# apple/ml-stable-diffusion

Measured on NVIDIA H100. Metric: diffusion_iter_per_s, higher is better.
Workload: dtype f16

## Files before the change

### ml-stable-diffusion_b200/csrc/common.cuh

```cuda
#pragma once

#include <cuda.h>
#include <cuda_fp16.h>
#include <cuda_runtime.h>
#include <stdint.h>
#include <stdio.h>
#include <string.h>

namespace b200sd {

void set_error(const char* fmt, ...);

#define B200SD_CHECK_CUDA(expr)                                                            \
    do {                                                                                   \
        cudaError_t _e = (expr);                                                           \
        if (_e != cudaSuccess) {                                                           \
            ::b200sd::set_error("%s failed: %s (%s:%d)", #expr, cudaGetErrorString(_e),    \
                                __FILE__, __LINE__);                                       \
            return 1;                                                                      \
        }                                                                                  \
    } while (0)

#define B200SD_REQUIRE(cond, ...)                                                          \
    do {                                                                                   \
// ... 255 lines not shown
        : "memory");
}

__device__ __forceinline__ void wgmma_m64n64_rs_tb(float* d, const uint32_t (&a)[4], uint64_t db, uint32_t acc) {
    asm volatile(
        "{\n\t.reg .pred p;\n\tsetp.ne.b32 p, %37, 0;\n\t"
        "wgmma.mma_async.sync.aligned.m64n64k16.f32.f16.f16 "
        "{%0, %1, %2, %3, %4, %5, %6, %7, %8, %9, %10, %11, %12, %13, %14, %15, "
        "%16, %17, %18, %19, %20, %21, %22, %23, %24, %25, %26, %27, %28, %29, %30, %31}, "
        "{%32, %33, %34, %35}, %36, p, 1, 1, 1;\n\t}\n"
        : B200SD_F8(0), B200SD_F8(8), B200SD_F8(16), B200SD_F8(24)
        : "r"(a[0]), "r"(a[1]), "r"(a[2]), "r"(a[3]), "l"(db), "r"(acc)
        : "memory");
}
template <int N>
__device__ __forceinline__ void wgmma_rs_tb(float* d, const uint32_t (&a)[4], uint64_t db, uint32_t acc);
template <>
__device__ __forceinline__ void wgmma_rs_tb<64>(float* d, const uint32_t (&a)[4], uint64_t db, uint32_t acc) {
    wgmma_m64n64_rs_tb(d, a, db, acc);
}
template <>
__device__ __forceinline__ void wgmma_rs_tb<128>(float* d, const uint32_t (&a)[4], uint64_t db, uint32_t acc) {
    asm volatile(
        "{\n\t.reg .pred p;\n\tsetp.ne.b32 p, %69, 0;\n\t"
        "wgmma.mma_async.sync.aligned.m64n128k16.f32.f16.f16 "
        "{%0, %1, %2, %3, %4, %5, %6, %7, %8, %9, %10, %11, %12, %13, %14, %15, "
        "%16, %17, %18, %19, %20, %21, %22, %23, %24, %25, %26, %27, %28, %29, %30, %31, "
        "%32, %33, %34, %35, %36, %37, %38, %39, %40, %41, %42, %43, %44, %45, %46, %47, "
        "%48, %49, %50, %51, %52, %53, %54, %55, %56, %57, %58, %59, %60, %61, %62, %63}, "
        "{%64, %65, %66, %67}, %68, p, 1, 1, 1;\n\t}\n"
        : B200SD_F8(0), B200SD_F8(8), B200SD_F8(16), B200SD_F8(24), B200SD_F8(32), B200SD_F8(40), B200SD_F8(48), B200SD_F8(56)
        : "r"(a[0]), "r"(a[1]), "r"(a[2]), "r"(a[3]), "l"(db), "r"(acc)
        : "memory");
}
template <>
__device__ __forceinline__ void wgmma_rs_tb<192>(float* d, const uint32_t (&a)[4], uint64_t db, uint32_t acc) {
    asm volatile(
        "{\n\t.reg .pred p;\n\tsetp.ne.b32 p, %101, 0;\n\t"
        "wgmma.mma_async.sync.aligned.m64n192k16.f32.f16.f16 "
        "{%0, %1, %2, %3, %4, %5, %6, %7, %8, %9, %10, %11, %12, %13, %14, %15, "
        "%16, %17, %18, %19, %20, %21, %22, %23, %24, %25, %26, %27, %28, %29, %30, %31, "
        "%32, %33, %34, %35, %36, %37, %38, %39, %40, %41, %42, %43, %44, %45, %46, %47, "
        "%48, %49, %50, %51, %52, %53, %54, %55, %56, %57, %58, %59, %60, %61, %62, %63, "
        "%64, %65, %66, %67, %68, %69, %70, %71, %72, %73, %74, %75, %76, %77, %78, %79, "
        "%80, %81, %82, %83, %84, %85, %86, %87, %88, %89, %90, %91, %92, %93, %94, %95}, "
        "{%96, %97, %98, %99}, %100, p, 1, 1, 1;\n\t}\n"
        : B200SD_F8(0), B200SD_F8(8), B200SD_F8(16), B200SD_F8(24), B200SD_F8(32), B200SD_F8(40), B200SD_F8(48), B200SD_F8(56),
          B200SD_F8(64), B200SD_F8(72), B200SD_F8(80), B200SD_F8(88)
        : "r"(a[0]), "r"(a[1]), "r"(a[2]), "r"(a[3]), "l"(db), "r"(acc)
        : "memory");
}
#undef B200SD_F8

template <int R>
__device__ __forceinline__ void wgmma_rows64(float (&d)[R], int bn, uint64_t da, uint64_t db, uint32_t acc) {
#pragma unroll
    for (int c = 0; c + 64 <= 2 * R; c += 64)
        if (c + 64 <= bn) wgmma_ss<64>(d + c / 2, da, db + (c * 128 >> 4), acc);
    const int c32 = bn & ~63;
#pragma unroll
    for (int c = 0; c + 32 <= 2 * R; c += 64)
        if (c == c32 && (bn & 32)) wgmma_ss<32>(d + c / 2, da, db + (c * 128 >> 4), acc);
    const int c16 = bn & ~31;
#pragma unroll
    for (int c = 0; c + 16 <= 2 * R; c += 32)
        if (c == c16 && (bn & 16)) wgmma_ss<16>(d + c / 2, da, db + (c * 128 >> 4), acc);
}

__device__ __forceinline__ uint64_t make_smem_desc_sw128(uint32_t smem_addr, uint32_t sbo_bytes, uint32_t lbo_bytes) {
    uint64_t d = 0;
    d |= static_cast<uint64_t>((smem_addr >> 4) & 0x3FFF);
    d |= static_cast<uint64_t>((lbo_bytes >> 4) & 0x3FFF) << 16;
    d |= static_cast<uint64_t>((sbo_bytes >> 4) & 0x3FFF) << 32;
    d |= static_cast<uint64_t>(1) << 62;
    return d;
}

__device__ __forceinline__ float ex2_approx(float x) {
    float y;
    asm("ex2.approx.ftz.f32 %0, %1;" : "=f"(y) : "f"(x));
    return y;
}

__device__ __forceinline__ float silu_f(float x) { return __fdividef(x, 1.0f + __expf(-x)); }
__device__ __forceinline__ float erf_as(float x) {
    const float ax = fabsf(x);
    float t;
    asm("rcp.approx.ftz.f32 %0, %1;" : "=f"(t) : "f"(fmaf(0.3275911f, ax, 1.0f)));
    float poly = fmaf(1.061405429f, t, -1.453152027f);
    poly = fmaf(poly, t, 1.421413741f);
    poly = fmaf(poly, t, -0.284496736f);
    poly = fmaf(poly, t, 0.254829592f);
    poly *= t;
    const float e = ex2_approx(-ax * ax * 1.4426950408889634f);
    const float r = fmaf(-poly, e, 1.0f);
    return copysignf(r, x);
}
__device__ __forceinline__ float gelu_erf_f(float x) { return 0.5f * x * (1.0f + erf_as(x * 0.70710678118654752f)); }

__device__ __forceinline__ uint32_t pack_half2(float a, float b) {
    __half2 h = __floats2half2_rn(a, b);
    return *reinterpret_cast<uint32_t*>(&h);
}
#endif

}
```

### ml-stable-diffusion_b200/csrc/gemm_conv.cu

```cuda
#include "common.cuh"
#include "../../include/b200sd.h"

#include <algorithm>
#include <cmath>
#include <stdlib.h>

namespace b200sd {

static constexpr int kBM = 128;
static constexpr int kBK = 64;
static constexpr int kAStage = kBM * kBK * 2;
static constexpr int kGemmThreads = 384;
static constexpr int kProducerRegs = 40;
static constexpr int kConsumerRegs = 232;
static constexpr int kHaloThreads = 288;
static constexpr int kEpiThreads = 256;
static constexpr int kProducerWarp = 8;
static constexpr int kMaxStages = 8;
static constexpr int kHaloMaxStages = 24;
static constexpr int kSmemBudget = 220 * 1024;
static constexpr int kEpiFixed = 2 * 256 * 4 + 256 * 4 + 64;

static int smem_budget() {
    const char* e = getenv("B200SD_SMEM_KB");
    if (e && e[0]) {
        const int kb = atoi(e);
        if (kb >= 48 && kb <= 220) return kb * 1024;
    }
    return kSmemBudget;
}

struct __align__(64) GemmParams {
    CUtensorMap tmA0, tmA1, tmB;
    CUtensorMap tmA2, tmA3;
    int kc2, kc3;
    int mode, M, N, n_store;
    int C0, Kpt, kc0, kc, taps;
    int kb_total, kb_per_split, splits;
    int m_tiles, n_tiles, block_n, stages;
    int n_img, Hout, Wout, stride, bw_log2, bh_log2, tiles_w, tiles_h;
    int bias_rows, bias_stride, geglu, out_f32;
    int act;
    int cluster;
    int pad_lo;
    int wgt_tiled;
    int bias_mode;
    int res_smem;
    void* out;
    const float* bias;
    const __half* residual;
    float* partial;
    int H, W, Wp, tiles_per_img, patch_rows, patch_bytes, upsample;
    int inv_wp;
    int win, tw, th, tiles_x;
    int desc_bo;
    int tma_patch, patch_tx;
    const __half* a0;
    const __half* a1;
    int C1;
    const float* gn_chan0;
    const float* gn_chan1;
    const float* gn_gamma;
    const float* gn_beta;
    int gn_groups, gn_silu, gn_hw;
    float gn_eps;
    float* cs_partial;
    float* cs_chan;
    unsigned int* cs_tickets;
// ... 784 lines not shown
                                for (int j = 0; j < 16; ++j) a16[j] = __uint_as_float(v[j]);
                                process16(a16, c);
                            }
                        }
                    }
                    if (!kPartial && p.rs_out != nullptr && valid)
                        *reinterpret_cast<float2*>(p.rs_out + (static_cast<size_t>(t.n_tile * 2 + half) * p.M + out_row) * 2) = rowacc;
                }
            }
            fence_proxy_async_smem();
            epi_bar_sync();
            if (threadIdx.x == 0) mbar_arrive(acc_free);
        }
        if (kPartial && p.cluster) {
            cluster_sync_all();
            cluster_splitk_reduce(p, smem, threadIdx.x);
            cluster_sync_all();
        }
    }
}


static constexpr int kGemmWidths[] = {256, 192, 160, 128, 96, 64, 32, 16};
static constexpr int kNumGemmWidths = sizeof(kGemmWidths) / sizeof(kGemmWidths[0]);
static int gemm_width_index(int bn) {
    for (int i = 0; i < kNumGemmWidths; ++i)
        if (kGemmWidths[i] == bn) return i;
    return -1;
}
using KernelFn = void (*)(GemmParams);
template <bool kGeneric, bool kGeglu, bool kOutF32, bool kPartial, bool kStaged>
static KernelFn gemm_kernel(int width_index) {
#define B200SD_GEMM_FN(bn) wgmma_gemm_kernel<kGeneric, kGeglu, kOutF32, kPartial, kStaged, bn>
    static const KernelFn fns[kNumGemmWidths] = {B200SD_GEMM_FN(256), B200SD_GEMM_FN(192), B200SD_GEMM_FN(160),
                                                 B200SD_GEMM_FN(128), B200SD_GEMM_FN(96),  B200SD_GEMM_FN(64),
                                                 B200SD_GEMM_FN(32),  B200SD_GEMM_FN(16)};
#undef B200SD_GEMM_FN
    return fns[width_index];
}

__device__ __forceinline__ float silu_fast(float y) {
    float th;
    asm("tanh.approx.f32 %0, %1;" : "=f"(th) : "f"(0.5f * y));
    const float hy = 0.5f * y;
    return fmaf(hy, th, hy);
}

__device__ __forceinline__ void dbg_mark(const GemmParams& p, int slot) {
    if (p.dbg != nullptr && blockIdx.x == 0) p.dbg[slot] = clock64();
}

__device__ __forceinline__ void ldr_bar_sync() { asm volatile("bar.sync 1, 256;" ::: "memory"); }

template <int kKind, int kR>
__global__ void __launch_bounds__(kHaloThreads, 1) halo_conv_kernel(const __grid_constant__ GemmParams p) {
    constexpr bool kFp32Direct = kKind == 1;
    constexpr bool kTmaPatch = kKind == 2;
    extern __shared__ __align__(1024) uint8_t smem_raw[];
    uint8_t* smem = smem_raw;
    if (threadIdx.x == 0 && (smem_u32(smem) & 1023u) != 0) __trap();
    const int b_stage = p.block_n * (kBK * 2);
    uint8_t* patch = smem;
    uint8_t* smem_b = smem + 2 * p.patch_bytes;
    uint64_t* full_b = reinterpret_cast<uint64_t*>(smem_b + p.stages * b_stage);
    uint64_t* empty_b = full_b + kHaloMaxStages;
    uint64_t* full_a = empty_b + kHaloMaxStages;
    uint64_t* empty_a = full_a + 2;
    uint64_t* acc_free = empty_a + 2;
    float* bias_s = reinterpret_cast<float*>(acc_free + 4);
    unsigned int* flag_s = reinterpret_cast<unsigned int*>(bias_s + 256);
    float2* stat_s = reinterpret_cast<float2*>(flag_s + 16);
    float2* scsh = stat_s + 64;
    const int Cin = p.C0 + p.C1;
    __half* stage_tile = reinterpret_cast<__half*>(scsh + ((Cin + 7) & ~7));
    float* acc_s = reinterpret_cast<float*>(smem);
    const int lda = p.block_n + 4;

    const int warp = threadIdx.x >> 5;
    const int lane = threadIdx.x & 31;
    if (warp == kProducerWarp && lane == 0) {
        prefetch_tmap(&p.tmB);
        if (kTmaPatch) {
            prefetch_tmap(&p.tmA0);
            prefetch_tmap(&p.tmA1);
        }
        for (int s = 0; s < p.stages; ++s) {
            mbar_init(&full_b[s], 1);
            mbar_init(&empty_b[s], 2);
        }
        for (int s = 0; s < 2; ++s) {
            mbar_init(&full_a[s], 1);
            mbar_init(&empty_a[s], 2);
        }
        mbar_init(acc_free, 1);
        fence_barrier_init();
    }
    __syncthreads();
    pdl_trigger();

    const int total_work = p.m_tiles * p.n_tiles;
    const int work0 = blockIdx.x, work_step = gridDim.x;
    const int kc = p.kc;

    if (warp == kProducerWarp) {
        if (lane == 0) {
            int it = 0, iter = 0;
            int ci = 0, pai = 0, pwork = work0, pj = 0;
            auto issue_patch = [&](bool blocking) -> bool {
                const int pa = pai & 1;
                const uint32_t ph = ((pai >> 1) & 1) ^ 1;
                if (blocking) mbar_wait(&empty_a[pa], ph);
                else if (!mbar_try_wait(&empty_a[pa], ph)) return false;
                const TileCoord pt = decode_work(p, pwork);
                const bool src1 = pj >= p.kc0;
                mbar_expect_tx(&full_a[pa], static_cast<uint32_t>(p.patch_tx));
                tma_load_4d(patch + pa * p.patch_bytes + 1024, src1 ? &p.tmA1 : &p.tmA0, &full_a[pa],
                            (src1 ? pj - p.kc0 : pj) * kBK, pt.xa, pt.ya, pt.n0, kEvictNormal);
                ++pai;
                if (++pj == kc) pj = 0, pwork += work_step;
                return true;
            };
            if (kTmaPatch) pdl_wait();
            for (int work = work0; work < total_work; work += work_step, ++iter) {
                const TileCoord t = decode_work(p, work);
                if (iter > 0) mbar_wait(acc_free, (iter - 1) & 1);
                for (int j = 0; j < kc; ++j, ++ci) {
                    if (kTmaPatch && pai == ci) issue_patch(true);
                    for (int tap = 0; tap < p.taps; ++tap, ++it) {
                        if (kTmaPatch && pai == ci + 1 && pwork == work) issue_patch(false);
                        const int st = it % p.stages;
                        const uint32_t ph = (it / p.stages) & 1;
                        mbar_wait(&empty_b[st], ph ^ 1);
                        mbar_expect_tx(&full_b[st], b_stage);
                        tma_load_2d(smem_b + st * b_stage, &p.tmB, &full_b[st], 0,
                                    (t.n_tile * p.kb_total + j * p.taps + tap) * p.block_n, kEvictFirst);
                    }
                }
            }
        }
    } else if (warp < kProducerWarp) {
        const int ltid = threadIdx.x;
        const int ew = warp;
        const int wg = warp >> 2;
        const int r0 = 64 * wg + 16 * (warp & 3) + (lane >> 2);
        const int row = (warp & 3) * 32 + lane;
        const bool leader = (threadIdx.x & 127) == 0;
        const bool gn = p.gn_gamma != nullptr;
        const bool ups = p.upsample != 0;
        const int Hs = ups ? (p.H >> 1) : p.H, Ws = ups ? (p.W >> 1) : p.W;
        float acc[kR];
        if (ltid == 0) dbg_mark(p, 0);
        pdl_wait();
        if (ltid == 0) dbg_mark(p, 1);
        int cur_img = -1, ait = 0, it = 0;
        for (int work = work0; work < total_work; work += work_step) {
            const TileCoord t = decode_work(p, work);
            const int img = t.n0;
            const int ya = t.ya, xa = t.xa;
            const int ncol0 = t.n_tile * p.block_n;
            if (p.bias != nullptr) {
                const float* bsrc = p.bias + (p.bias_rows > 0 ? static_cast<size_t>(img) * p.bias_stride : 0);
                for (int c = ltid; c < p.block_n; c += kEpiThreads) bias_s[c] = (ncol0 + c < p.N) ? bsrc[ncol0 + c] : 0.f;
            }
            if (ltid < 16) {
                const int which = ltid >> 3;
                *reinterpret_cast<uint4*>(patch + which * p.patch_bytes + 7 * 128 + (ltid & 7) * 16) = make_uint4(0, 0, 0, 0);
            }
            constexpr int NBMAX = kTmaPatch ? 1 : 12;
            const int nvec = p.patch_rows * p.Wp * 8;
            const int nb = (nvec + kEpiThreads - 1) / kEpiThreads;
            const int jj = ltid & 7;
            int soff[NBMAX], doff[NBMAX];
            uint4 regs[NBMAX];
            auto chunk_src = [&](int j, int& csrc) -> const __half* {
                const bool src1 = j >= p.kc0;
                const int cbase = (src1 ? j - p.kc0 : j) * kBK + jj * 8;
                csrc = src1 ? p.C1 : p.C0;
                if (cbase >= csrc) return nullptr;
                return (src1 ? p.a1 : p.a0) + static_cast<size_t>(img) * Hs * Ws * csrc + cbase;
            };
            float4 cf[4];
            bool chan_ok = false;
            int csrc_nxt = 0;
            const __half* nsrc = nullptr;
            auto transform_begin = [&](int tj) {
                const bool src1 = tj >= p.kc0;
                int csrc_cur;
                chan_ok = chunk_src(tj, csrc_cur) != nullptr;
                nsrc = (tj + 1 < kc) ? chunk_src(tj + 1, csrc_nxt) : nullptr;
                if (gn) {
                    const float2* tab = scsh + (src1 ? p.C0 : 0) + (src1 ? tj - p.kc0 : tj) * kBK + jj * 8;
#pragma unroll
                    for (int q = 0; q < 4; ++q) cf[q] = chan_ok ? *reinterpret_cast<const float4*>(tab + 2 * q) : make_float4(0.f, 0.f, 0.f, 0.f);
                }
            };
            auto transform_slice = [&](int pa, int slice, int nslices) {
                uint8_t* pbase = patch + pa * p.patch_bytes + 1024;
#pragma unroll
                for (int i = 0; i < NBMAX; ++i) {
                    if (doff[i] < 0 || i % nslices != slice) continue;
                    uint4 val = regs[i];
                    const bool live = soff[i] >= 0;
                    regs[i] = make_uint4(0, 0, 0, 0);
                    if (nsrc != nullptr && live)
                        regs[i] = __ldg(reinterpret_cast<const uint4*>(nsrc + static_cast<size_t>(soff[i]) * csrc_nxt));
                    if (gn && live && chan_ok) {
                        __half2* h2 = reinterpret_cast<__half2*>(&val);
#pragma unroll
                        for (int q = 0; q < 4; ++q) {
                            const float2 f = __half22float2(h2[q]);
                            float a = fmaf(f.x, cf[q].x, cf[q].y), b = fmaf(f.y, cf[q].z, cf[q].w);
                            if (p.gn_silu) a = silu_fast(a), b = silu_fast(b);
                            h2[q] = __floats2half2_rn(a, b);
                        }
                    }
                    *reinterpret_cast<uint4*>(pbase + doff[i]) = val;
                }
            };
            if (!kTmaPatch) {
#pragma unroll
                for (int i = 0; i < NBMAX; ++i) {
                    const int v = ltid + kEpiThreads * i;
                    const int pi = v >> 3;
                    const int prow = (pi * p.inv_wp) >> 20;
                    const int yy = ya + prow, xx = xa + (pi - prow * p.Wp);
                    const bool in_patch = i < nb && v < nvec;
                    const bool ok = in_patch && yy >= 0 && yy < p.H && xx >= 0 && xx < p.W;
                    const int ys = ups ? (yy >> 1) : yy, xs = ups ? (xx >> 1) : xx;
                    soff[i] = ok ? (ys * Ws + xs) : -1;
                    doff[i] = in_patch ? pi * 128 + ((jj ^ (pi & 7)) << 4) : -1;
                }
                {
                    int csrc;
                    const __half* src = chunk_src(0, csrc);
#pragma unroll
                    for (int i = 0; i < NBMAX; ++i) {
                        regs[i] = make_uint4(0, 0, 0, 0);
                        if (src != nullptr && soff[i] >= 0)
                            regs[i] = __ldg(reinterpret_cast<const uint4*>(src + static_cast<size_t>(soff[i]) * csrc));
                    }
                }
                if (ltid == 0) dbg_mark(p, 2);
                if (gn && img != cur_img) {
                    const int cpg = Cin / p.gn_groups;
                    const float inv_cnt = 1.0f / (static_cast<float>(cpg) * static_cast<float>(p.gn_hw));
                    ldr_bar_sync();
                    for (int g = ltid >> 3; g < p.gn_groups; g += kEpiThreads >> 3) {
                        float s = 0.f, q = 0.f;
                        for (int c = g * cpg + (ltid & 7); c < (g + 1) * cpg; c += 8) {
                            const float2 v = (c < p.C0)
                                ? __ldg(reinterpret_cast<const float2*>(p.gn_chan0 + (static_cast<size_t>(img) * p.C0 + c) * 2))
                                : __ldg(reinterpret_cast<const float2*>(p.gn_chan1 + (static_cast<size_t>(img) * p.C1 + c - p.C0) * 2));
                            s += v.x, q += v.y;
                        }
#pragma unroll
                        for (int o = 4; o > 0; o >>= 1) {
                            s += __shfl_xor_sync(0xffffffffu, s, o);
                            q += __shfl_xor_sync(0xffffffffu, q, o);
                        }
                        if ((ltid & 7) == 0) {
                            const float mean = s * inv_cnt;
                            stat_s[g] = make_float2(mean, rsqrtf(fmaxf(q * inv_cnt - mean * mean, 0.f) + p.gn_eps));
                        }
                    }
                    ldr_bar_sync();
                    for (int c = ltid; c < Cin; c += kEpiThreads) {
                        const float2 st = stat_s[c / cpg];
                        const float sc = p.gn_gamma[c] * st.y;
                        scsh[c] = make_float2(sc, fmaf(-st.x, sc, p.gn_beta[c]));
                    }
                    ldr_bar_sync();
                    cur_img = img;
                }
                if (ltid == 0) dbg_mark(p, 8);
                transform_begin(0);
                transform_slice(ait & 1, 0, 1);
            }
            fence_proxy_async_smem();
            epi_bar_sync();
            if (ltid == 0) {
                if (!kTmaPatch) dbg_mark(p, 9);
                dbg_mark(p, 3);
            }
            for (int j = 0; j < kc; ++j, ++ait) {
                const int pa = ait & 1;
                if (kTmaPatch) mbar_wait(&full_a[pa], (ait >> 1) & 1);
                const bool more = !kTmaPatch && j + 1 < kc;
                if (ltid == 0 && j < 24) dbg_mark(p, 64 + 2 * j);
                if (more) {
                    if (ltid == 0 && j < 23) dbg_mark(p, 10 + 2 * j);
                    transform_begin(j + 1);
                }
                const uint32_t pbase = smem_u32(patch + pa * p.patch_bytes) + 1024;
                int prev = -1;
                for (int tap = 0; tap < p.taps; ++tap, ++it) {
                    const int st = it % p.stages;
                    mbar_wait(&full_b[st], (it / p.stages) & 1);
                    const int dy = p.taps == 9 ? tap / 3 - 1 : 0, dx = p.taps == 9 ? tap - (tap / 3) * 3 - 1 : 0;
                    const int srow = t.c0 + dy * p.Wp + dx + 64 * wg;
                    const uint32_t a_addr = pbase + srow * 128;
                    const uint64_t adesc = make_smem_desc_sw128(a_addr, 1024, 0) |
                                           (static_cast<uint64_t>(p.desc_bo ? ((a_addr >> 7) & 7) : 0) << 49);
                    const uint64_t bdesc = make_smem_desc_sw128(smem_u32(smem_b + st * b_stage), 1024, 0);
                    wgmma_fence();
#pragma unroll
                    for (int k = 0; k < kBK / 16; ++k)
                        wgmma_rows64(acc, p.block_n, adesc + 2 * k, bdesc + 2 * k, (j > 0 || tap > 0 || k > 0) ? 1u : 0u);
                    wgmma_commit();
                    if (more) transform_slice(pa ^ 1, tap, p.taps);
                    wgmma_wait<1>();
                    if (prev >= 0 && leader) mbar_arrive(&empty_b[prev]);
                    prev = st;
                }
                wgmma_wait<0>();
                wgmma_fence_regs<kR>(acc);
                if (ltid == 0 && j < 24) dbg_mark(p, 65 + 2 * j);
                if (leader) {
                    mbar_arrive(&empty_b[prev]);
                    if (kTmaPatch) mbar_arrive(&empty_a[pa]);
                }
                if (more) {
                    fence_proxy_async_smem();
                    epi_bar_sync();
                    if (ltid == 0 && j < 23) dbg_mark(p, 11 + 2 * j);
                }
            }
            int out_row;
            const bool valid = tile_row(p, t, row, out_row);
            uint4 res_pre[4];
            if (kKind == 0) staged_load_residual(p, t, staged_map(p, t, lane), ew, 0, res_pre);
            epi_bar_sync();
            if (ltid == 0) dbg_mark(p, 4);
            if (kKind == 0) {
                __half* tile_s = p.stage_dedicated ? stage_tile : reinterpret_cast<__half*>(smem);
                float* scratch = reinterpret_cast<float*>(tile_s + kBM * (p.block_n + 8));
                const float* bias = p.bias != nullptr ? bias_s : nullptr;
                stage_accumulators(p, t, acc, tile_s, bias, bias, bias_s, r0, lane);
                staged_epilogue(p, t, tile_s, scratch, flag_s, ew, lane, res_pre);
            } else {
                park_accumulators(acc, p.block_n, acc_s, lda, r0, lane);
                epi_bar_sync();
                const float* arow = acc_s + row * lda;
                if (kFp32Direct) {
                    if (ew < 4) {
                        uint32_t v[16];
                        acc_ld16(arow, v);
                        if (valid) {
                            for (int c = 0; c < 16 && ncol0 + c < p.N; ++c) {
                                const float x = __uint_as_float(v[c]) + (p.bias != nullptr ? bias_s[c] : 0.f);
                                if (p.out_f32) reinterpret_cast<float*>(p.out)[static_cast<size_t>(out_row) * p.N + ncol0 + c] = x;
                                else reinterpret_cast<__half*>(p.out)[static_cast<size_t>(out_row) * p.N + ncol0 + c] = __float2half_rn(x);
                            }
                        }
                    }
                } else {
                    const int half = ew >> 2;
                    float2 rowacc = make_float2(0.f, 0.f);
                    for (int c = 32 * half; c < p.block_n && valid; c += 64) {
                        uint32_t v[32];
                        acc_ld32(arow + c, v);
#pragma unroll
                        for (int hh = 0; hh < 2; ++hh) {
                            const int cc = c + 16 * hh;
                            if (ncol0 + cc < p.N) {
                                float a16[16];
#pragma unroll
                                for (int q = 0; q < 16; ++q) a16[q] = __uint_as_float(v[16 * hh + q]);
                                const float* bptr = p.bias != nullptr ? bias_s + cc : nullptr;
                                const __half* rptr = p.residual != nullptr
                                    ? p.residual + static_cast<size_t>(out_row) * p.n_store + ncol0 + cc : nullptr;
                                epilogue_store16<true, false, false, false>(p, a16, out_row, ncol0 + cc, 0, bptr, rptr, rowacc);
                            }
                        }
                    }
                }
            }
            fence_proxy_async_smem();
            epi_bar_sync();
            if (ltid == 0) {
                dbg_mark(p, 5);
                mbar_arrive(acc_free);
            }
        }
    }
}

__global__ void splitk_reduce_kernel(const float* __restrict__ partial, int splits, int M, int N,
                                     const float* __restrict__ bias, int bias_rows, int bias_stride,
                                     const __half* __restrict__ residual, void* __restrict__ out, int out_f32) {
    pdl_wait();
    const size_t total4 = static_cast<size_t>(M) * N / 4;
    const size_t stride = static_cast<size_t>(M) * N;
    for (size_t i = blockIdx.x * static_cast<size_t>(blockDim.x) + threadIdx.x; i < total4;
         i += static_cast<size_t>(gridDim.x) * blockDim.x) {
        const size_t e = i * 4;
        float4 acc = *reinterpret_cast<const float4*>(partial + e);
        for (int s = 1; s < splits; ++s) {
            const float4 v = *reinterpret_cast<const float4*>(partial + s * stride + e);
            acc.x += v.x, acc.y += v.y, acc.z += v.z, acc.w += v.w;
        }
        const int row = static_cast<int>(e / N);
        const int col = static_cast<int>(e - static_cast<size_t>(row) * N);
        if (bias != nullptr) {
            const float* b = bias + (bias_rows > 0 ? (row / bias_rows) * bias_stride : 0) + col;
            acc.x += b[0], acc.y += b[1], acc.z += b[2], acc.w += b[3];
        }
        if (residual != nullptr) {
            const __half2* r = reinterpret_cast<const __half2*>(residual + e);
            const float2 r0 = __half22float2(r[0]), r1 = __half22float2(r[1]);
            acc.x += r0.x, acc.y += r0.y, acc.z += r1.x, acc.w += r1.y;
        }
        if (out_f32) {
            *reinterpret_cast<float4*>(reinterpret_cast<float*>(out) + e) = acc;
        } else {
            uint2 pk;
            pk.x = pack_half2(acc.x, acc.y);
            pk.y = pack_half2(acc.z, acc.w);
            *reinterpret_cast<uint2*>(reinterpret_cast<__half*>(out) + e) = pk;
        }
    }
}

struct GemmPlan {
    int M, N, Kpt, taps, kc0, kc1, kb_total;
    int m_tiles, n_tiles, block_n, splits, kb_per_split, stages;
    int Hout, Wout, bw, bh, bn_img, tiles_w, tiles_h, tiles_n;
    int bias_mode, res_smem, epi_smem;
    int cluster;
    int halo;
    int Wp, tiles_per_img, patch_rows, patch_bytes;
    int win, tw, th, tiles_x;
    int staged, stage_dedicated;
    int tma_patch;
    int cs_slots;
    int smem_bytes;
    int variant;
    int halo_kind;
};

// ... 13 lines not shown
}

static bool staged_enabled() {
    const char* e = getenv("B200SD_STAGED");
    return e && e[0] == '1';
}

static bool desc_base_offset_enabled() {
    const char* e = getenv("B200SD_DESC_BO");
    return e && e[0] == '1';
}

static int plan_halo(const b200sd_gemm_args& a, GemmPlan& pl) {
    B200SD_REQUIRE((a.mode == 0 || a.stride == 1) && !a.pad_after_only, "b200sd_gemm: halo needs a stride-1 pad-1 convolution");
    B200SD_REQUIRE(!a.geglu && a.act == 0 && a.split_k <= 1, "b200sd_gemm: halo kernel: no GEGLU / activation / split-K");
    B200SD_REQUIRE(a.wgt_tiled && a.block_n > 0, "b200sd_gemm: halo kernel needs chunk-major pre-tiled weights (explicit block_n)");
    B200SD_REQUIRE(a.n_img > 0 && a.h > 0 && a.w > 0, "b200sd_gemm: bad image geometry for the halo kernel");
    B200SD_REQUIRE(!a.upsample2x || (a.h % 2 == 0 && a.w % 2 == 0 && a.c1 == 0 && a.gn_groups == 0),
                   "b200sd_gemm: upsample2x needs even output size, one source, no GroupNorm");
    pl.halo = 1;
    pl.tma_patch = a.halo == 2 ? 1 : 0;
    B200SD_REQUIRE(!pl.tma_patch || (a.gn_groups == 0 && !a.upsample2x && a.cs_partial == nullptr && !a.out_f32 &&
                                     a.block_n % 32 == 0 && a.c0 % 8 == 0 && a.c1 % 8 == 0),
                   "b200sd_gemm: halo = 2 (TMA patches) is the plain convolution: no GroupNorm / upsample / statistics / fp32 output");
    pl.bw = pl.bh = pl.bn_img = pl.tiles_w = pl.tiles_h = pl.tiles_n = 1;
    pl.Hout = a.h, pl.Wout = a.w;
    pl.M = a.n_img * a.h * a.w;
    const bool conv = a.mode == 1;
    const int halo = conv ? 1 : 0;
    pl.win = 0, pl.tw = pl.th = pl.tiles_x = 0;
    if (a.w + 1 <= 80) {
        pl.Wp = a.w + 1;
        pl.tiles_per_img = (a.h * pl.Wp + kBM - 1) / kBM;
        const int span = (kBM - 1 + pl.Wp - 1) / pl.Wp + 1;
        pl.patch_rows = span + 2 * halo;
    } else {
        double best = -1.0;
        for (int th = 1; th <= 8; th *= 2) {
            const int pitch = kBM / th, tw = pitch - 2 * halo;
            const int tx = (a.w + tw - 1) / tw, ty = (a.h + th - 1) / th;
            const double eff = static_cast<double>(a.w) * a.h / (static_cast<double>(tx) * ty * kBM);
            if (eff > best) best = eff, pl.th = th, pl.tw = tw, pl.tiles_x = tx, pl.tiles_per_img = tx * ty;
        }
        pl.win = 1;
        pl.Wp = pl.tw + 2 * halo;
        pl.patch_rows = pl.th + 2 * halo;
    }
    pl.m_tiles = a.n_img * pl.tiles_per_img;
    const int rows_needed = std::max(pl.patch_rows * pl.Wp, (2 * halo + 1) * pl.Wp + kBM) + 8 + 1;
    pl.patch_bytes = ((rows_needed + 7) / 8) * 1024;
    B200SD_REQUIRE(pl.tma_patch || pl.patch_rows * pl.Wp * 8 <= 12 * kEpiThreads, "b200sd_gemm: image too wide for the halo kernel's patch (w=%d)", a.w);
    B200SD_REQUIRE(!pl.tma_patch || (pl.Wp <= 256 && pl.patch_rows <= 256), "b200sd_gemm: patch exceeds a TMA box (w=%d)", a.w);
    pl.block_n = a.block_n;
    B200SD_REQUIRE(pl.block_n == 16 || (pl.block_n % 32 == 0 && pl.block_n <= 256), "b200sd_gemm: halo block_n %d", pl.block_n);
    pl.n_tiles = (a.n + pl.block_n - 1) / pl.block_n;
    pl.splits = 1, pl.kb_per_split = pl.kb_total, pl.cluster = 0;
    pl.bias_mode = a.bias != nullptr ? 1 : 0;
    pl.res_smem = 0;
    const bool fp32_direct = a.out_f32 || pl.block_n == 16;
    B200SD_REQUIRE(!fp32_direct || (pl.block_n == 16 && a.residual == nullptr && a.cs_partial == nullptr),
                   "b200sd_gemm: halo fp32 / narrow output needs block_n 16, no residual, no statistics");
    pl.staged = (fp32_direct || pl.tma_patch) ? 0 : 1;
    B200SD_REQUIRE(pl.tma_patch || pl.block_n <= 128, "b200sd_gemm: halo block_n %d > 128 needs halo = 2", pl.block_n);
    pl.stage_dedicated = 0;
    const int cin = a.c0 + a.c1;
    const int fixed = 2 * pl.patch_bytes + (2 * kHaloMaxStages + 8) * 8 + 16 + 256 * 4 + 64 + 64 * 8 + ((cin + 7) & ~7) * 8 +
                      (pl.stage_dedicated ? kBM * (pl.block_n + 8) * 2 + 8 * pl.block_n * 8 : 0) + 1024;
    const int b_stage = pl.block_n * kBK * 2;
    pl.stages = std::min(kHaloMaxStages, (227 * 1024 - fixed) / b_stage);
    B200SD_REQUIRE(pl.stages >= 3, "b200sd_gemm: halo kernel does not fit shared memory (w=%d c=%d block_n=%d)", a.w, cin, pl.block_n);
    pl.smem_bytes = fixed + pl.stages * b_stage;
    const int over = 2 * pl.patch_bytes + pl.stages * b_stage;
    B200SD_REQUIRE(over >= (pl.staged ? kBM * (pl.block_n + 8) * 2 + 8 * pl.block_n * 8 : kBM * (pl.block_n + 4) * 4),
                   "b200sd_gemm: halo epilogue tile does not fit over the pipeline memory (block_n=%d)", pl.block_n);
    pl.epi_smem = 0;
    pl.cs_slots = pl.tiles_per_img;
    pl.variant = -1;
    pl.halo_kind = pl.tma_patch ? 2 : (pl.staged == 0 ? 1 : 0);
    return 0;
}

static int halo_pick_block_n(const b200sd_gemm_args& a) {
    if (a.n <= 16) return 16;
    const int wp = a.w + 1;
    long m_tiles = static_cast<long>(a.n_img) * ((a.h * wp + kBM - 1) / kBM);
    if (wp > 80) m_tiles = static_cast<long>(a.n_img) * ((static_cast<long>(a.h) * a.w + 101) / 102);
    double best = 1e30;
    int best_bn = 128;
    for (int bn = a.halo == 2 ? 256 : 128; bn >= 32; bn -= 32) {
        const int nt = (a.n + bn - 1) / bn;
        if (nt * bn > a.n + a.n / 4 + 31) continue;
        const double waves = std::ceil(static_cast<double>(m_tiles * nt) / num_sms());
        const double t = waves * ((41.0 + bn / 2.0) * (a.mode == 1 ? 36.0 : 4.0) * ((a.c0 + a.c1 + 63) / 64) + 4000.0) + 2.0 * nt;
        if (t < best) best = t, best_bn = bn;
    }
    return best_bn;
}

static int plan_gemm(const b200sd_gemm_args& a, GemmPlan& pl) {
    B200SD_REQUIRE(a.mode == 0 || a.mode == 1, "b200sd_gemm: bad mode %d", a.mode);
    B200SD_REQUIRE(!a.pad_after_only || (a.mode == 1 && a.stride == 2), "b200sd_gemm: pad_after_only is for stride-2 convolutions");
    B200SD_REQUIRE(a.c0 > 0 && a.c0 % 8 == 0 && a.c1 >= 0 && a.c1 % 8 == 0,
                   "b200sd_gemm: channel counts must be positive multiples of 8 (c0=%d c1=%d)", a.c0, a.c1);
    B200SD_REQUIRE(a.n > 0, "b200sd_gemm: n=%d", a.n);
    pl.N = a.n;
    pl.Kpt = a.c0 + a.c1;
    pl.kc0 = (a.c0 + kBK - 1) / kBK;
    pl.kc1 = (a.c1 + kBK - 1) / kBK;
    pl.taps = a.mode == 1 ? 9 : 1;
    pl.kb_total = pl.taps * (pl.kc0 + pl.kc1) + (a.c2 + kBK - 1) / kBK + (a.c3 + kBK - 1) / kBK;
    B200SD_REQUIRE((a.c2 == 0 && a.c3 == 0) || (a.mode == 1 && a.stride == 1 && !a.halo && a.c2 > 0 && a.c2 % 8 == 0 && a.c3 % 8 == 0),
                   "b200sd_gemm: shortcut sources (a2 / a3) need a stride-1 3x3 convolution and channel counts that are multiples of 8");
    pl.halo = 0, pl.Wp = 0, pl.tiles_per_img = 0, pl.patch_rows = 0, pl.patch_bytes = 0;
    pl.staged = 0, pl.stage_dedicated = 0, pl.cs_slots = 0, pl.smem_bytes = 0;
    const bool want_stats = a.cs_partial != nullptr || a.rs_out != nullptr;
    B200SD_REQUIRE(!want_stats || (!a.geglu && !a.out_f32 && a.act == 0 && a.n % 8 == 0 && a.split_k <= 1),
                   "b200sd_gemm: statistics outputs need a plain fp16 epilogue without split-K");
    B200SD_REQUIRE(a.ln_parts == 0 || (a.mode == 0 && a.ln_stat && a.ln_wg && a.split_k <= 1),
                   "b200sd_gemm: LayerNorm fold needs mode 0, statistics, the fold vector and no split-K");
    if (a.halo) return plan_halo(a, pl);
    if (a.mode == 0) {
        B200SD_REQUIRE(a.m > 0, "b200sd_gemm: m=%d", a.m);
        pl.M = a.m;
        pl.m_tiles = (a.m + kBM - 1) / kBM;
        pl.Hout = pl.Wout = pl.bw = pl.bh = pl.bn_img = pl.tiles_w = pl.tiles_h = pl.tiles_n = 1;
    } else {
        B200SD_REQUIRE(a.stride == 1 || a.stride == 2, "b200sd_gemm: stride %d", a.stride);
        B200SD_REQUIRE(a.n_img > 0 && a.h > 0 && a.w > 0, "b200sd_gemm: bad image geometry");
        B200SD_REQUIRE(a.stride == 1 || (a.h % 2 == 0 && a.w % 2 == 0), "b200sd_gemm: stride-2 needs even h, w");
        pl.Hout = a.h / a.stride;
        pl.Wout = a.w / a.stride;
        pl.M = a.n_img * pl.Hout * pl.Wout;
        long best = -1;
        for (int bw = 128; bw >= 1; bw >>= 1) {
            if (bw * a.stride > 256) continue;
            for (int bh = 128 / bw; bh >= 1; bh >>= 1) {
                if (bh * a.stride > 256) continue;
                const int bn = 128 / (bw * bh);
                const int tw = (pl.Wout + bw - 1) / bw, th = (pl.Hout + bh - 1) / bh, tn = (a.n_img + bn - 1) / bn;
                const long tiles = static_cast<long>(tw) * th * tn;
                const long score = tiles * 1024 - bw;
                if (best < 0 || score < best) {
// ... 223 lines not shown
    p.m_tiles = pl.m_tiles;
    p.n_tiles = pl.n_tiles;
    p.block_n = pl.block_n;
    p.stages = pl.stages;
    p.n_img = a.n_img;
    p.Hout = pl.Hout;
    p.Wout = pl.Wout;
    p.stride = a.mode == 1 ? a.stride : 1;
    p.bw_log2 = ilog2(pl.bw);
    p.bh_log2 = ilog2(pl.bh);
    p.tiles_w = pl.tiles_w;
    p.tiles_h = pl.tiles_h;
    p.bias_rows = a.bias_rows;
    p.bias_stride = a.bias_stride > 0 ? a.bias_stride : a.n;
    p.geglu = a.geglu;
    p.out_f32 = a.out_f32;
    p.act = a.act;
    p.pad_lo = a.pad_after_only ? 0 : 1;
    p.wgt_tiled = a.wgt_tiled;
    p.bias_mode = pl.bias_mode;
    p.res_smem = pl.res_smem;
    p.out = a.out;
    p.bias = a.bias;
    p.residual = reinterpret_cast<const __half*>(a.residual);
    p.partial = (pl.splits > 1 && !pl.cluster) ? a.workspace : nullptr;
    p.cluster = pl.cluster;
    p.H = a.h, p.W = a.w, p.Wp = pl.Wp, p.tiles_per_img = pl.tiles_per_img;
    p.win = pl.win, p.tw = pl.tw, p.th = pl.th, p.tiles_x = pl.tiles_x;
    p.inv_wp = pl.Wp > 0 ? (1 << 20) / pl.Wp + 1 : 0;
    p.patch_rows = pl.patch_rows, p.patch_bytes = pl.patch_bytes;
    p.upsample = a.upsample2x, p.desc_bo = desc_base_offset_enabled() ? 1 : 0;
    p.tma_patch = pl.tma_patch, p.patch_tx = pl.patch_rows * pl.Wp * kBK * 2;
    p.a0 = reinterpret_cast<const __half*>(a.a0), p.a1 = reinterpret_cast<const __half*>(a.a1), p.C1 = a.c1;
    if (pl.halo && a.gn_groups > 0) {
        B200SD_REQUIRE(a.gn_chan0 && a.gn_gamma && a.gn_beta && (a.c1 == 0 || a.gn_chan1) && a.gn_groups <= 64 &&
                           (a.c0 + a.c1) % a.gn_groups == 0,
                       "b200sd_gemm: bad fused GroupNorm arguments");
        p.gn_chan0 = a.gn_chan0, p.gn_chan1 = a.gn_chan1, p.gn_gamma = a.gn_gamma, p.gn_beta = a.gn_beta;
        p.gn_groups = a.gn_groups, p.gn_silu = a.gn_silu, p.gn_eps = a.gn_eps, p.gn_hw = a.h * a.w;
    }
    p.cs_partial = a.cs_partial, p.cs_chan = a.cs_chan, p.cs_tickets = a.cs_tickets;
    p.cs_slots = pl.cs_slots;
    p.cs_hw = a.mode == 0 ? a.cs_hw : pl.Hout * pl.Wout;
    if (p.cs_hw <= 0) p.cs_hw = 1;
    B200SD_REQUIRE(a.cs_partial == nullptr || (a.cs_chan && a.cs_tickets), "b200sd_gemm: statistics outputs need cs_chan and cs_tickets");
    p.rs_out = a.rs_out;
    p.ln_stat = a.ln_stat, p.ln_wg = a.ln_wg, p.ln_parts = a.ln_parts, p.ln_eps = a.ln_eps, p.ln_k = a.c0 + a.c1;
    p.staged = pl.staged, p.stage_dedicated = pl.stage_dedicated;
    {
        const char* e = getenv("B200SD_DBG_PTR");
        p.dbg = (e && e[0]) ? reinterpret_cast<long long*>(strtoull(e, nullptr, 0)) : nullptr;
    }
    if (pl.halo) {
        using HaloFn = void (*)(GemmParams);
        const int kind = pl.halo_kind;
        const bool wide = pl.block_n > 128;
        HaloFn hfn = kind == 2 ? (wide ? halo_conv_kernel<2, 128> : halo_conv_kernel<2, 64>)
                               : (kind == 1 ? halo_conv_kernel<1, 8> : halo_conv_kernel<0, 64>);
        const int hslot = kind == 2 && wide ? 3 : kind;
        static bool hattr[4] = {false, false, false, false};
        if (!hattr[hslot]) {
            B200SD_CHECK_CUDA(cudaFuncSetAttribute(hfn, cudaFuncAttributeMaxDynamicSharedMemorySize, 227 * 1024));
            hattr[hslot] = true;
        }
        const int units = pl.m_tiles * pl.n_tiles;
        B200SD_CHECK_CUDA(launch_kernel(hfn, dim3(std::min(units, num_sms())), dim3(kHaloThreads), pl.smem_bytes, stream, p));
        B200SD_CHECK_CUDA(cudaGetLastError());
        count_launch(1);
        return 0;
    }

    const int smem_bytes = pl.smem_bytes;
    const int total = pl.m_tiles * pl.n_tiles * pl.splits;
    const int grid = std::min(total, num_sms());
    B200SD_REQUIRE(a.act == 0 || (a.act >= 1 && a.act <= 3 && pl.splits == 1 && !a.geglu), "b200sd_gemm: act=%d unsupported here", a.act);
    const int wi = gemm_width_index(pl.block_n);
    const int variant = pl.variant;
    KernelFn fn;
    switch (variant) {
        case kVariantGeneric: fn = gemm_kernel<true, false, false, false, false>(wi); break;
        case kVariantStaged: fn = gemm_kernel<false, false, false, false, true>(wi); break;
        case kVariantSplitK: fn = gemm_kernel<false, false, false, true, false>(wi); break;
        case kVariantGeglu: fn = gemm_kernel<false, true, false, false, false>(wi); break;
        case kVariantF32: fn = gemm_kernel<false, false, true, false, false>(wi); break;
        default: fn = gemm_kernel<false, false, false, false, false>(wi); break;
    }
    if (pl.splits > 1 && !pl.cluster) {
        p.bias = nullptr;
        p.residual = nullptr;
    }
    static bool attr_set[6][kNumGemmWidths] = {};
    if (!attr_set[variant][wi]) {
        B200SD_CHECK_CUDA(cudaFuncSetAttribute(fn, cudaFuncAttributeMaxDynamicSharedMemorySize, 227 * 1024));
        attr_set[variant][wi] = true;
    }
    if (pl.cluster) {
        B200SD_REQUIRE(variant == 1, "b200sd_gemm: cluster split-K needs the regular epilogue variant");
        cudaLaunchConfig_t cfg;
        memset(&cfg, 0, sizeof(cfg));
        cfg.gridDim = dim3(total);
        cfg.blockDim = dim3(kGemmThreads);
        cfg.dynamicSmemBytes = smem_bytes;
        cfg.stream = stream;
        cudaLaunchAttribute at[2];
        at[0].id = cudaLaunchAttributeClusterDimension;
        at[0].val.clusterDim.x = pl.splits;
        at[0].val.clusterDim.y = 1;
        at[0].val.clusterDim.z = 1;
        cfg.attrs = at;
        cfg.numAttrs = 1;
        if (pdl_enabled()) {
            at[1].id = cudaLaunchAttributeProgrammaticStreamSerialization;
            at[1].val.programmaticStreamSerializationAllowed = 1;
            cfg.numAttrs = 2;
        }
        B200SD_CHECK_CUDA(cudaLaunchKernelEx(&cfg, fn, p));
        B200SD_CHECK_CUDA(cudaGetLastError());
        count_launch(1);
        return 0;
// ... 73 lines not shown
```

Measured before the change: 141.6.

## Specialize halo conv kernel per block_n and keep wgmma chain in flight across k-chunks

The halo convolution kernel is templated on the exact block_n so each tap issues a single wgmma of full width, replacing the runtime-dispatched chain of 64/32/16 pieces. The kernel now launches with 384 threads and uses setmaxnreg to move registers from producer warps to consumer warps. The per-chunk wgmma_wait<0> drain is removed: the next patch is transformed once after the first tap, guarded by a new patch_free barrier, and accumulators drain only once per tile. This adds many template instantiations (binary size and compile time) and new synchronisation on patch reuse, which carries ordering risk.

```diff
diff --git a/ml-stable-diffusion_b200/csrc/common.cuh b/ml-stable-diffusion_b200/csrc/common.cuh
--- a/ml-stable-diffusion_b200/csrc/common.cuh
+++ b/ml-stable-diffusion_b200/csrc/common.cuh
@@ -331,21 +331,6 @@
 }
 #undef B200SD_F8
 
-template <int R>
-__device__ __forceinline__ void wgmma_rows64(float (&d)[R], int bn, uint64_t da, uint64_t db, uint32_t acc) {
-#pragma unroll
-    for (int c = 0; c + 64 <= 2 * R; c += 64)
-        if (c + 64 <= bn) wgmma_ss<64>(d + c / 2, da, db + (c * 128 >> 4), acc);
-    const int c32 = bn & ~63;
-#pragma unroll
-    for (int c = 0; c + 32 <= 2 * R; c += 64)
-        if (c == c32 && (bn & 32)) wgmma_ss<32>(d + c / 2, da, db + (c * 128 >> 4), acc);
-    const int c16 = bn & ~31;
-#pragma unroll
-    for (int c = 0; c + 16 <= 2 * R; c += 32)
-        if (c == c16 && (bn & 16)) wgmma_ss<16>(d + c / 2, da, db + (c * 128 >> 4), acc);
-}
-
 __device__ __forceinline__ uint64_t make_smem_desc_sw128(uint32_t smem_addr, uint32_t sbo_bytes, uint32_t lbo_bytes) {
     uint64_t d = 0;
     d |= static_cast<uint64_t>((smem_addr >> 4) & 0x3FFF);
diff --git a/ml-stable-diffusion_b200/csrc/gemm_conv.cu b/ml-stable-diffusion_b200/csrc/gemm_conv.cu
--- a/ml-stable-diffusion_b200/csrc/gemm_conv.cu
+++ b/ml-stable-diffusion_b200/csrc/gemm_conv.cu
@@ -13,7 +13,6 @@
 static constexpr int kGemmThreads = 384;
 static constexpr int kProducerRegs = 40;
 static constexpr int kConsumerRegs = 232;
-static constexpr int kHaloThreads = 288;
 static constexpr int kEpiThreads = 256;
 static constexpr int kProducerWarp = 8;
 static constexpr int kMaxStages = 8;
@@ -904,8 +903,8 @@
 
 __device__ __forceinline__ void ldr_bar_sync() { asm volatile("bar.sync 1, 256;" ::: "memory"); }
 
-template <int kKind, int kR>
-__global__ void __launch_bounds__(kHaloThreads, 1) halo_conv_kernel(const __grid_constant__ GemmParams p) {
+template <int kKind, int kBN>
+__global__ void __launch_bounds__(kGemmThreads, 1) halo_conv_kernel(const __grid_constant__ GemmParams p) {
     constexpr bool kFp32Direct = kKind == 1;
     constexpr bool kTmaPatch = kKind == 2;
     extern __shared__ __align__(1024) uint8_t smem_raw[];
@@ -918,6 +917,7 @@
     uint64_t* empty_b = full_b + kHaloMaxStages;
     uint64_t* full_a = empty_b + kHaloMaxStages;
     uint64_t* empty_a = full_a + 2;
+    uint64_t* patch_free = empty_a;
     uint64_t* acc_free = empty_a + 2;
     float* bias_s = reinterpret_cast<float*>(acc_free + 4);
     unsigned int* flag_s = reinterpret_cast<unsigned int*>(bias_s + 256);
@@ -954,8 +954,9 @@
     const int work0 = blockIdx.x, work_step = gridDim.x;
     const int kc = p.kc;
 
-    if (warp == kProducerWarp) {
-        if (lane == 0) {
+    if (warp >= kProducerWarp) {
+        setmaxnreg_dec<kProducerRegs>();
+        if (warp == kProducerWarp && lane == 0) {
             int it = 0, iter = 0;
             int ci = 0, pai = 0, pwork = work0, pj = 0;
             auto issue_patch = [&](bool blocking) -> bool {
@@ -990,7 +991,8 @@
                 }
             }
         }
-    } else if (warp < kProducerWarp) {
+    } else {
+        setmaxnreg_inc<kConsumerRegs>();
         const int ltid = threadIdx.x;
         const int ew = warp;
         const int wg = warp >> 2;
@@ -1000,11 +1002,12 @@
         const bool gn = p.gn_gamma != nullptr;
         const bool ups = p.upsample != 0;
         const int Hs = ups ? (p.H >> 1) : p.H, Ws = ups ? (p.W >> 1) : p.W;
-        float acc[kR];
+        float acc[kBN / 2];
         if (ltid == 0) dbg_mark(p, 0);
         pdl_wait();
         if (ltid == 0) dbg_mark(p, 1);
         int cur_img = -1, ait = 0, it = 0;
+        uint32_t pf_phase = 0;
         for (int work = work0; work < total_work; work += work_step) {
             const TileCoord t = decode_work(p, work);
             const int img = t.n0;
@@ -1046,11 +1049,11 @@
                     for (int q = 0; q < 4; ++q) cf[q] = chan_ok ? *reinterpret_cast<const float4*>(tab + 2 * q) : make_float4(0.f, 0.f, 0.f, 0.f);
                 }
             };
-            auto transform_slice = [&](int pa, int slice, int nslices) {
+            auto transform_chunk = [&](int pa) {
                 uint8_t* pbase = patch + pa * p.patch_bytes + 1024;
 #pragma unroll
                 for (int i = 0; i < NBMAX; ++i) {
-                    if (doff[i] < 0 || i % nslices != slice) continue;
+                    if (doff[i] < 0) continue;
                     uint4 val = regs[i];
                     const bool live = soff[i] >= 0;
                     regs[i] = make_uint4(0, 0, 0, 0);
@@ -1126,7 +1129,7 @@
                 }
                 if (ltid == 0) dbg_mark(p, 8);
                 transform_begin(0);
-                transform_slice(ait & 1, 0, 1);
+                transform_chunk(ait & 1);
             }
             fence_proxy_async_smem();
             epi_bar_sync();
@@ -1134,6 +1137,7 @@
                 if (!kTmaPatch) dbg_mark(p, 9);
                 dbg_mark(p, 3);
             }
+            int prev = -1;
             for (int j = 0; j < kc; ++j, ++ait) {
                 const int pa = ait & 1;
                 if (kTmaPatch) mbar_wait(&full_a[pa], (ait >> 1) & 1);
@@ -1144,7 +1148,6 @@
                     transform_begin(j + 1);
                 }
                 const uint32_t pbase = smem_u32(patch + pa * p.patch_bytes) + 1024;
-                int prev = -1;
                 for (int tap = 0; tap < p.taps; ++tap, ++it) {
                     const int st = it % p.stages;
                     mbar_wait(&full_b[st], (it / p.stages) & 1);
@@ -1157,25 +1160,35 @@
                     wgmma_fence();
 #pragma unroll
                     for (int k = 0; k < kBK / 16; ++k)
-                        wgmma_rows64(acc, p.block_n, adesc + 2 * k, bdesc + 2 * k, (j > 0 || tap > 0 || k > 0) ? 1u : 0u);
+                        wgmma_ss<kBN>(acc, adesc + 2 * k, bdesc + 2 * k, (j > 0 || tap > 0 || k > 0) ? 1u : 0u);
                     wgmma_commit();
-                    if (more) transform_slice(pa ^ 1, tap, p.taps);
+                    if (tap == 0 && j > 0) {
+                        wgmma_wait<1>();
+                        if (kTmaPatch) {
+                            if (leader) mbar_arrive(&empty_a[pa ^ 1]);
+                        } else if (more) {
+                            if (leader) mbar_arrive(patch_free);
+                            mbar_wait(patch_free, pf_phase);
+                            pf_phase ^= 1;
+                        }
+                    }
+                    if (more && tap == 0) transform_chunk(pa ^ 1);
                     wgmma_wait<1>();
                     if (prev >= 0 && leader) mbar_arrive(&empty_b[prev]);
                     prev = st;
                 }
-                wgmma_wait<0>();
-                wgmma_fence_regs<kR>(acc);
                 if (ltid == 0 && j < 24) dbg_mark(p, 65 + 2 * j);
-                if (leader) {
-                    mbar_arrive(&empty_b[prev]);
-                    if (kTmaPatch) mbar_arrive(&empty_a[pa]);
-                }
                 if (more) {
                     fence_proxy_async_smem();
                     epi_bar_sync();
                     if (ltid == 0 && j < 23) dbg_mark(p, 11 + 2 * j);
                 }
+            }
+            wgmma_wait<0>();
+            wgmma_fence_regs<kBN / 2>(acc);
+            if (leader) {
+                mbar_arrive(&empty_b[prev]);
+                if (kTmaPatch) mbar_arrive(&empty_a[(ait - 1) & 1]);
             }
             int out_row;
             const bool valid = tile_row(p, t, row, out_row);
@@ -1237,6 +1250,22 @@
     }
 }
 
+static constexpr int kHaloLoaderMaxBN = 192;
+static bool halo_width_compiled(int kind, int bn) {
+    if (kind == 1) return bn == 16;
+    return bn >= 32 && gemm_width_index(bn) >= 0 && (kind == 2 || bn <= kHaloLoaderMaxBN);
+}
+static KernelFn halo_kernel(int kind, int width_index) {
+#define B200SD_HALO_FNS(k) halo_conv_kernel<k, 192>, halo_conv_kernel<k, 160>, halo_conv_kernel<k, 128>, \
+                           halo_conv_kernel<k, 96>, halo_conv_kernel<k, 64>, halo_conv_kernel<k, 32>, nullptr
+    static const KernelFn fns[3][kNumGemmWidths] = {
+        {nullptr, B200SD_HALO_FNS(0)},
+        {nullptr, nullptr, nullptr, nullptr, nullptr, nullptr, nullptr, halo_conv_kernel<1, 16>},
+        {halo_conv_kernel<2, 256>, B200SD_HALO_FNS(2)}};
+#undef B200SD_HALO_FNS
+    return (kind >= 0 && kind < 3 && width_index >= 0) ? fns[kind][width_index] : nullptr;
+}
+
 __global__ void splitk_reduce_kernel(const float* __restrict__ partial, int splits, int M, int N,
                                      const float* __restrict__ bias, int bias_rows, int bias_stride,
                                      const __half* __restrict__ residual, void* __restrict__ out, int out_f32) {
@@ -1356,7 +1385,6 @@
     B200SD_REQUIRE(pl.tma_patch || pl.patch_rows * pl.Wp * 8 <= 12 * kEpiThreads, "b200sd_gemm: image too wide for the halo kernel's patch (w=%d)", a.w);
     B200SD_REQUIRE(!pl.tma_patch || (pl.Wp <= 256 && pl.patch_rows <= 256), "b200sd_gemm: patch exceeds a TMA box (w=%d)", a.w);
     pl.block_n = a.block_n;
-    B200SD_REQUIRE(pl.block_n == 16 || (pl.block_n % 32 == 0 && pl.block_n <= 256), "b200sd_gemm: halo block_n %d", pl.block_n);
     pl.n_tiles = (a.n + pl.block_n - 1) / pl.block_n;
     pl.splits = 1, pl.kb_per_split = pl.kb_total, pl.cluster = 0;
     pl.bias_mode = a.bias != nullptr ? 1 : 0;
@@ -1365,7 +1393,9 @@
     B200SD_REQUIRE(!fp32_direct || (pl.block_n == 16 && a.residual == nullptr && a.cs_partial == nullptr),
                    "b200sd_gemm: halo fp32 / narrow output needs block_n 16, no residual, no statistics");
     pl.staged = (fp32_direct || pl.tma_patch) ? 0 : 1;
-    B200SD_REQUIRE(pl.tma_patch || pl.block_n <= 128, "b200sd_gemm: halo block_n %d > 128 needs halo = 2", pl.block_n);
+    pl.halo_kind = pl.tma_patch ? 2 : (pl.staged == 0 ? 1 : 0);
+    B200SD_REQUIRE(halo_width_compiled(pl.halo_kind, pl.block_n), "b200sd_gemm: halo kind %d is not compiled for block_n %d",
+                   pl.halo_kind, pl.block_n);
     pl.stage_dedicated = 0;
     const int cin = a.c0 + a.c1;
     const int fixed = 2 * pl.patch_bytes + (2 * kHaloMaxStages + 8) * 8 + 16 + 256 * 4 + 64 + 64 * 8 + ((cin + 7) & ~7) * 8 +
@@ -1380,7 +1410,6 @@
     pl.epi_smem = 0;
     pl.cs_slots = pl.tiles_per_img;
     pl.variant = -1;
-    pl.halo_kind = pl.tma_patch ? 2 : (pl.staged == 0 ? 1 : 0);
     return 0;
 }
 
@@ -1391,7 +1420,8 @@
     if (wp > 80) m_tiles = static_cast<long>(a.n_img) * ((static_cast<long>(a.h) * a.w + 101) / 102);
     double best = 1e30;
     int best_bn = 128;
-    for (int bn = a.halo == 2 ? 256 : 128; bn >= 32; bn -= 32) {
+    for (int bn : kGemmWidths) {
+        if (!halo_width_compiled(a.halo == 2 ? 2 : 0, bn)) continue;
         const int nt = (a.n + bn - 1) / bn;
         if (nt * bn > a.n + a.n / 4 + 31) continue;
         const double waves = std::ceil(static_cast<double>(m_tiles * nt) / num_sms());
@@ -1721,19 +1751,16 @@
         p.dbg = (e && e[0]) ? reinterpret_cast<long long*>(strtoull(e, nullptr, 0)) : nullptr;
     }
     if (pl.halo) {
-        using HaloFn = void (*)(GemmParams);
-        const int kind = pl.halo_kind;
-        const bool wide = pl.block_n > 128;
-        HaloFn hfn = kind == 2 ? (wide ? halo_conv_kernel<2, 128> : halo_conv_kernel<2, 64>)
-                               : (kind == 1 ? halo_conv_kernel<1, 8> : halo_conv_kernel<0, 64>);
-        const int hslot = kind == 2 && wide ? 3 : kind;
-        static bool hattr[4] = {false, false, false, false};
-        if (!hattr[hslot]) {
+        const int wi = gemm_width_index(pl.block_n);
+        const KernelFn hfn = halo_kernel(pl.halo_kind, wi);
+        B200SD_REQUIRE(hfn != nullptr, "b200sd_gemm: halo kind %d is not compiled for block_n %d", pl.halo_kind, pl.block_n);
+        static bool hattr[3][kNumGemmWidths] = {};
+        if (!hattr[pl.halo_kind][wi]) {
             B200SD_CHECK_CUDA(cudaFuncSetAttribute(hfn, cudaFuncAttributeMaxDynamicSharedMemorySize, 227 * 1024));
-            hattr[hslot] = true;
+            hattr[pl.halo_kind][wi] = true;
         }
         const int units = pl.m_tiles * pl.n_tiles;
-        B200SD_CHECK_CUDA(launch_kernel(hfn, dim3(std::min(units, num_sms())), dim3(kHaloThreads), pl.smem_bytes, stream, p));
+        B200SD_CHECK_CUDA(launch_kernel(hfn, dim3(std::min(units, num_sms())), dim3(kGemmThreads), pl.smem_bytes, stream, p));
         B200SD_CHECK_CUDA(cudaGetLastError());
         count_launch(1);
         return 0;
```

Result: no change. 140.9, median of 6 (-0.5%).
